# AliBahri94/GM3D

Measured on AMD Instinct MI355X. Metric: point-clouds/sec pretrain step (N=1024,G=64), higher is better.
Workload: dtype bf16

## Files before the change

### gm3d_amd/csrc/gemm_ws.hip

```cpp
#include "mfma.hpp"

namespace gm3d {

__device__ __forceinline__ void ws_wait_vm(int n) {
#define GM3D_WS_CASE(N_) case N_: asm volatile("s_waitcnt vmcnt(%0)" ::"n"(N_) : "memory"); break;
    switch (n) {
        GM3D_WS_CASE(0) GM3D_WS_CASE(4) GM3D_WS_CASE(8) GM3D_WS_CASE(12) GM3D_WS_CASE(16) GM3D_WS_CASE(24) GM3D_WS_CASE(32)
        GM3D_WS_CASE(36) GM3D_WS_CASE(48)
        default: asm volatile("s_waitcnt vmcnt(0)" ::: "memory"); break;
    }
#undef GM3D_WS_CASE
}

struct WsBn {
    const bf16_t* T;
    const float* scale;
    const float* shift;
    float* partial;
    int ldt;
    float slope;
};

constexpr int ws_depth(int ppl, int tile, int stage) {
    int d = 48 / ppl < 4 ? 48 / ppl : 4;
    while (d > 1 && (d + 1) * tile + stage > 152 * 1024) --d;
    return d;
}

template <int KT, int NW, int NL, int EPI, int TM>
__global__ __launch_bounds__(64 * (NW + NL)) void gemm_tn_ws_kernel(const bf16_t* __restrict__ A, const bf16_t* __restrict__ W,
                                                                     const float* __restrict__ bias, bf16_t* __restrict__ C, int M, int N,
                                                                     int lda, int ldw, int ldc, int tiles_n, bf16_t* __restrict__ P,
                                                                     uint8_t* __restrict__ ARG, int ldp, int bias_after_pool, WsBn bn,
                                                                     int Kreal, int pool16) {
    extern __shared__ __attribute__((aligned(16))) unsigned char wsm[];
    constexpr int BN = 32 * NW, NIMG = BN / 64 > 0 ? (BN + 63) / 64 : 1;
    constexpr int HALF = KT * 4096;
    constexpr int TILE = TM * HALF;
    constexpr int NP = TM * 4 * KT;
    constexpr int PPL = NP / NL;
    constexpr int STAGE = TM * NIMG * 4096;
    constexpr int DEPTH = ws_depth(PPL, TILE, STAGE);
    constexpr int NT = DEPTH + 1;
    static_assert(NP % NL == 0 && PPL <= 48, "loader split");
    unsigned char* stage = wsm + NT * TILE;
    const int tid = threadIdx.x, lane = tid & 63, w = __builtin_amdgcn_readfirstlane(tid >> 6);
    const int r = lane & 31, hh = lane >> 5;
    const int logical = xcd_tile(blockIdx.x, gridDim.x);
    const int tile_n = logical % tiles_n, first = logical / tiles_n, stride = gridDim.x / tiles_n;
    const int tiles_m = (M + 32 * TM - 1) / (32 * TM);
    const int nmine = first < tiles_m ? (tiles_m - first + stride - 1) / stride : 0;
    const int n0 = tile_n * BN;
    const unsigned lds0 = lds_addr(wsm);

    if (w >= NW) {
        const int lw = w - NW, prow = lane >> 3, pslot = lane & 7;
        auto issue = [&](int i) {
            const int m0 = (first + i * stride) * (32 * TM);
            const unsigned base = lds0 + (i % NT) * TILE;
#pragma unroll
            for (int q = 0; q < PPL; ++q) {
                const int p = lw * PPL + q, t = p / (4 * KT), pp = p - t * (4 * KT), kt = pp >> 2, row = 8 * (pp & 3) + prow;
                const int gr = m0 + 32 * t + row;
                const int am = gr < M ? gr : M - 1;
                int col = 64 * kt + ((pslot ^ swz(row)) << 3);
                col = col < Kreal ? col : 0;
                glds16(A + (size_t)am * lda + col, base + 1024 * p);
            }
        };
        for (int d = 0; d < DEPTH && d < nmine; ++d) issue(d);
        for (int i = 0; i < nmine; ++i) {
            if (i + DEPTH < nmine) issue(i + DEPTH);
            const int ahead = nmine - 1 - i < DEPTH ? nmine - 1 - i : DEPTH;
            ws_wait_vm(ahead * PPL);
            __builtin_amdgcn_s_barrier();
            __builtin_amdgcn_s_barrier();
        }
        return;
    }

    bf16x8 wreg[KT][4];
    {
        const bf16_t* wp = W + (size_t)(n0 + 32 * w + r) * ldw + 8 * hh;
#pragma unroll
        for (int kt = 0; kt < KT; ++kt)
#pragma unroll
            for (int s = 0; s < 4; ++s) {
                if (64 * kt + 16 * s + 8 * hh < Kreal) wreg[kt][s] = *reinterpret_cast<const bf16x8*>(wp + 64 * kt + 16 * s);
                else
#pragma unroll
                    for (int e = 0; e < 8; ++e) wreg[kt][s][e] = (bf16_t)0.0f;
            }
    }
    float bq[4][4];
#pragma unroll
    for (int q = 0; q < 4; ++q)
#pragma unroll
        for (int e = 0; e < 4; ++e) bq[q][e] = (EPI != 3 && bias) ? bias[n0 + 32 * w + 8 * q + 4 * hh + e] : 0.f;
    const float bcol = (EPI == 3 && bias) ? bias[n0 + 32 * w + r] : 0.f;
    const bool bias_in_tile = EPI != 3 || !bias_after_pool;
    float bn_a[4][4], bn_b[4][4];
    if (EPI == 4 || EPI == 5) {
#pragma unroll
        for (int q = 0; q < 4; ++q)
#pragma unroll
            for (int e = 0; e < 4; ++e) {
                const int col = n0 + 32 * w + 8 * q + 4 * hh + e;
                bn_a[q][e] = EPI == 4 ? bn.scale[col] : 0.f;
                bn_b[q][e] = EPI == 4 ? bn.shift[col] : 0.f;
            }
    }
    constexpr int CTHREADS = 64 * NW;

    for (int i = 0; i < nmine; ++i) {
        const int m0 = (first + i * stride) * (32 * TM);
        float tq[TM][4][4];
        if (EPI == 4 || EPI == 5) {
            typedef const __attribute__((address_space(4))) unsigned int* sptr_t;
#pragma unroll
            for (int t = 0; t < TM; ++t) {
                const size_t trow = pool16 ? (size_t)2 * ((m0 >> 5) + t) : (size_t)((m0 >> 5) + t);
                sptr_t tp = (sptr_t)(const void*)(bn.T + trow * bn.ldt + n0 + 32 * w);
                unsigned tw[16];
#pragma unroll
                for (int j = 0; j < 16; ++j) tw[j] = tp[j];
                if (pool16) {
                    sptr_t tp2 = (sptr_t)(const void*)(bn.T + (trow + 1) * bn.ldt + n0 + 32 * w);
                    unsigned tw2[16];
#pragma unroll
                    for (int j = 0; j < 16; ++j) tw2[j] = tp2[j];
                    if (r & 16) {
#pragma unroll
                        for (int j = 0; j < 16; ++j) tw[j] = tw2[j];
                    }
                }
#pragma unroll
                for (int q = 0; q < 4; ++q)
#pragma unroll
                    for (int e2 = 0; e2 < 2; ++e2) {
                        const unsigned u = hh ? tw[4 * q + 2 + e2] : tw[4 * q + e2];
                        tq[t][q][2 * e2] = __builtin_bit_cast(float, u << 16);
                        tq[t][q][2 * e2 + 1] = __builtin_bit_cast(float, u & 0xffff0000u);
                    }
            }
        }
        __builtin_amdgcn_s_barrier();
        const unsigned char* as = wsm + (i % NT) * TILE;
        f32x16 acc[TM];
#pragma unroll
        for (int t = 0; t < TM; ++t)
#pragma unroll
            for (int g = 0; g < 16; ++g) acc[t][g] = 0.f;
#pragma unroll
        for (int kt = 0; kt < KT; ++kt) {
            bf16x8 fa[TM][4];
#pragma unroll
            for (int t = 0; t < TM; ++t)
#pragma unroll
                for (int s = 0; s < 4; ++s) fa[t][s] = *reinterpret_cast<const bf16x8*>(as + t * HALF + kt * 4096 + swz_off(r, 2 * s + hh));
#pragma unroll
            for (int s = 0; s < 4; ++s)
#pragma unroll
                for (int t = 0; t < TM; ++t)
                    acc[t] = EPI == 3 ? mfma_bf16(fa[t][s], wreg[kt][s], acc[t])
                                      : mfma_bf16(wreg[kt][s], fa[t][s], acc[t]);
        }
        if (EPI == 3 && !C) __builtin_amdgcn_s_barrier();
        if (EPI == 3) {
            unsigned short rowbits[TM][16];
#pragma unroll
            for (int t = 0; t < TM; ++t) {
                unsigned best = 0, best2 = 0;
#pragma unroll
                for (int g = 0; g < 16; ++g) {
                    const bf16_t o = (bf16_t)(acc[t][g] + (bias_in_tile ? bcol : 0.f));
                    rowbits[t][g] = __builtin_bit_cast(unsigned short, o);
                    unsigned u = (unsigned)rowbits[t][g] << 16;
                    u = u == 0x80000000u ? 0u : u;
                    const unsigned k = (u ^ (unsigned)(((int)u >> 31) | (int)0x80000000)) & 0xffff0000u;
                    const unsigned key = k | (unsigned)(31 - (8 * (g >> 2) + 4 * hh + (g & 3)));
                    if (pool16 && g >= 8) best2 = key > best2 ? key : best2;
                    else best = key > best ? key : best;
                }
                {
                    const unsigned other = (unsigned)__shfl_xor((int)best, 32);
                    best = other > best ? other : best;
                    const unsigned other2 = (unsigned)__shfl_xor((int)best2, 32);
                    best2 = other2 > best2 ? other2 : best2;
                }
                if (hh == 0 && m0 + 32 * t < M) {
                    const unsigned k = best & 0xffff0000u;
                    const unsigned u = (k & 0x80000000u) ? (k & 0x7fff0000u) : (~k & 0xffff0000u);
                    float v = __builtin_bit_cast(float, u);
                    if (bias_after_pool) v += bcol;
                    if (!pool16) {
                        const size_t o = (size_t)((m0 >> 5) + t) * ldp + n0 + 32 * w + r;
                        P[o] = (bf16_t)v;
                        ARG[o] = (uint8_t)(31u - (best & 0xffu));
                    } else {
                        const size_t o = (size_t)((m0 >> 4) + 2 * t) * ldp + n0 + 32 * w + r;
                        P[o] = (bf16_t)v;
                        ARG[o] = (uint8_t)(31u - (best & 0xffu));
                        if (m0 + 32 * t + 16 < M) {
                            const unsigned k2 = best2 & 0xffff0000u;
                            const unsigned u2 = (k2 & 0x80000000u) ? (k2 & 0x7fff0000u) : (~k2 & 0xffff0000u);
                            float v2 = __builtin_bit_cast(float, u2);
                            if (bias_after_pool) v2 += bcol;
                            P[o + ldp] = (bf16_t)v2;
                            ARG[o + ldp] = (uint8_t)(15u - (best2 & 0xffu));
                        }
                    }
                }
            }
            if (!C) continue;
            const int ch = (((32 * w) & 63) + r) >> 3, sub = 2 * (r & 7);
#pragma unroll
            for (int t = 0; t < TM; ++t) {
                unsigned char* img = stage + (t * NIMG + ((32 * w) >> 6)) * 4096;
#pragma unroll
                for (int g = 0; g < 16; ++g) {
                    const int row = 8 * (g >> 2) + 4 * hh + (g & 3);
                    *reinterpret_cast<unsigned short*>(img + swz_off(row, ch) + sub) = rowbits[t][g];
                }
            }
        } else {
            const int cbase = ((32 * w) & 63) >> 3;
#pragma unroll
            for (int t = 0; t < TM; ++t) {
                unsigned char* img = stage + (t * NIMG + ((32 * w) >> 6)) * 4096;
#pragma unroll
                for (int q = 0; q < 4; ++q) {
                    bf16x4 pk;
#pragma unroll
                    for (int e = 0; e < 4; ++e) {
                        pk[e] = (bf16_t)(acc[t][4 * q + e] + bq[q][e]);
                        if (EPI == 4) {
                            const float h = ((float)pk[e] + tq[t][q][e]) * bn_a[q][e] + bn_b[q][e];
                            pk[e] = (bf16_t)(h > 0.f ? h : bn.slope * h);
                        }
                        if (EPI == 5) {
                            const float y = (float)pk[e] + tq[t][q][e];
                            bn_a[q][e] += y;
                            bn_b[q][e] += y * y;
                        }
                    }
                    *reinterpret_cast<bf16x4*>(img + swz_off(r, cbase + q) + 8 * hh) = pk;
                }
            }
        }
        asm volatile("s_waitcnt lgkmcnt(0)" ::: "memory");
        __builtin_amdgcn_s_barrier();
        {
            constexpr int CH = BN / 8;
#pragma unroll
            for (int c0 = 0; c0 < 32 * TM * CH; c0 += CTHREADS) {
                const int c = c0 + tid;
                if (c < 32 * TM * CH) {
                    const int row = c / CH, chunk = c - row * CH;
                    if (m0 + row < M) {
                        const uint4 raw = *reinterpret_cast<const uint4*>(stage + ((row >> 5) * NIMG + (chunk >> 3)) * 4096 + swz_off(row & 31, chunk & 7));
                        *reinterpret_cast<uint4*>(C + (size_t)(m0 + row) * ldc + n0 + 8 * chunk) = raw;
                    }
                }
            }
        }
    }
    if (EPI == 5) {
#pragma unroll
        for (int q = 0; q < 4; ++q)
#pragma unroll
            for (int e = 0; e < 4; ++e) {
#pragma unroll
                for (int m = 1; m < 32; m <<= 1) {
                    bn_a[q][e] += __shfl_xor(bn_a[q][e], m);
                    bn_b[q][e] += __shfl_xor(bn_b[q][e], m);
                }
                if (r == 0) {
                    const int col = n0 + 32 * w + 8 * q + 4 * hh + e;
                    bn.partial[(size_t)first * 2 * N + col] = bn_a[q][e];
                    bn.partial[(size_t)first * 2 * N + N + col] = bn_b[q][e];
                }
            }
    }
}

}

using gm3d::ws_depth;

static int ws_grid(int tiles_m, int tiles_n, size_t lds) {
    long long want = (long long)tiles_m * tiles_n;
    const int cap = 2 * lds <= 160 * 1024 ? 512 : 256;
    int g = want < cap ? (int)want : cap;
    g = (g + 7) / 8 * 8;
    while (g % tiles_n) g += 8;
    return g;
}

static int ws_launch(const void* A, const void* W, const float* bias, void* C, void* P, uint8_t* ARG, int M, int N, int K, int lda,
                     int ldw, int ldc, int ldp, int bias_after_pool, gm3d_stream_t stream, int bn_mode = 0, gm3d::WsBn bn = gm3d::WsBn(),
                     int pool16 = 0) {
    using namespace gm3d;
    if (!A || !W || (!C && !P) || M < 0 || N < 1 || K < 1) return GM3D_EINVAL;
    if (P && (!ARG || M % (pool16 ? 16 : 32) || ldp % 8 || ldp < N || ((size_t)ARG & 7) || ((size_t)P & 15))) return GM3D_EINVAL;
    if (K % 8 || K > 512 || lda % 8 || ldw % 8 || lda < K || ldw < K || (C && (ldc % 8 || ldc < N))) return GM3D_EUNSUPPORTED;
    if (((size_t)A | (size_t)W | (size_t)C) & 15) return GM3D_EUNSUPPORTED;
    if (M == 0) return GM3D_OK;
#define GM3D_WS_LAUNCH(KT, NW, NL, EPI, TM)                                                                               \
    {                                                                                                                    \
        constexpr int TILE_ = TM * KT * 4096, STAGE_ = TM * ((32 * NW + 63) / 64) * 4096;                                \
        constexpr int DEPTH_ = ws_depth(TM * 4 * KT / NL, TILE_, STAGE_);                                                \
        const size_t lds = (size_t)(DEPTH_ + 1) * TILE_ + STAGE_;                                                        \
        const int tiles_m = (M + 32 * TM - 1) / (32 * TM);                                                               \
        const int tiles_n = N / (32 * NW), grid = ws_grid(tiles_m, tiles_n, lds);                                        \
        return launch_lds<gemm_tn_ws_kernel<KT, NW, NL, EPI, TM>>(dim3(grid), dim3(64 * (NW + NL)), lds, stream, (const bf16_t*)A, \
                                                                  (const bf16_t*)W, bias, (bf16_t*)C, M, N, lda, ldw, ldc, tiles_n, \
                                                                  (bf16_t*)P, ARG, ldp, bias_after_pool, bn, K, pool16);        \
    }
    if (P) {
        if (K == 128 && N == 256) GM3D_WS_LAUNCH(2, 8, 1, 3, 1)
        if (K == 512 && N == 384) GM3D_WS_LAUNCH(8, 6, 2, 3, 1)
        if (K == 512 && N == 96) GM3D_WS_LAUNCH(8, 3, 2, 3, 1)
        return GM3D_EUNSUPPORTED;
    }
    if (bn_mode) {
        if (M % 32 || !bn.T || bn.ldt % 4 || bn.ldt < N || ((size_t)bn.T & 7)) return GM3D_EINVAL;
        if (K == 256 && N == 512 && bn_mode == 4) GM3D_WS_LAUNCH(4, 8, 1, 4, 1)
        if (K == 256 && N == 512 && bn_mode == 5) GM3D_WS_LAUNCH(4, 8, 1, 5, 1)
        return GM3D_EUNSUPPORTED;
    }
    if (K == 256 && N == 512) GM3D_WS_LAUNCH(4, 8, 1, 0, 1)
    if (K == 512 && N == 256) GM3D_WS_LAUNCH(8, 4, 2, 0, 1)
    if (K == 384 && N == 512) GM3D_WS_LAUNCH(6, 8, 2, 0, 1)
    if (K == 256 && N == 128) GM3D_WS_LAUNCH(4, 4, 1, 0, 1)
    if (K == 128 && N == 256) GM3D_WS_LAUNCH(2, 8, 1, 0, 1)
    if (K == 512 && N == 384) GM3D_WS_LAUNCH(8, 6, 2, 0, 1)
    if (K == 96 && N == 288) GM3D_WS_LAUNCH(2, 9, 1, 0, 1)
    if (K == 96 && N == 96) GM3D_WS_LAUNCH(2, 3, 1, 0, 1)
    if (K == 96 && N == 512) GM3D_WS_LAUNCH(2, 8, 1, 0, 1)
    if (K == 96 && N == 192) GM3D_WS_LAUNCH(2, 6, 1, 0, 1)
    if (K == 192 && N == 96) GM3D_WS_LAUNCH(3, 3, 1, 0, 1)
    if (K == 96 && N == 384) GM3D_WS_LAUNCH(2, 6, 1, 0, 1)
    if (K == 384 && N == 96) GM3D_WS_LAUNCH(6, 3, 1, 0, 1)
    if (K == 288 && N == 96) GM3D_WS_LAUNCH(5, 3, 1, 0, 1)
#undef GM3D_WS_LAUNCH
    return GM3D_EUNSUPPORTED;
}

extern "C" int gm3d_gemm_tn_bf16_ws(const void* A, const void* W, const float* bias, void* C, int M, int N, int K, int lda, int ldw,
                                    int ldc, gm3d_stream_t stream) {
    if (!C) return GM3D_EINVAL;
    return ws_launch(A, W, bias, C, nullptr, nullptr, M, N, K, lda, ldw, ldc, 0, 0, stream);
}

extern "C" int gm3d_gemm_tn_bf16_ws_pool(const void* A, const void* W, const float* bias, void* C, void* P, uint8_t* arg, int M, int N,
                                         int K, int lda, int ldw, int ldc, int ldp, int bias_after_pool, gm3d_stream_t stream) {
    if (!P || !arg) return GM3D_EINVAL;
    return ws_launch(A, W, bias, C, P, arg, M, N, K, lda, ldw, ldc, ldp, bias_after_pool, stream);
}

extern "C" int gm3d_gemm_tn_bf16_ws_poolg(const void* A, const void* W, const float* bias, void* C, void* P, uint8_t* arg, int M, int N,
                                          int K, int lda, int ldw, int ldc, int ldp, int bias_after_pool, int group_rows,
                                          gm3d_stream_t stream) {
    if (!P || !arg || (group_rows != 16 && group_rows != 32)) return GM3D_EINVAL;
    return ws_launch(A, W, bias, C, P, arg, M, N, K, lda, ldw, ldc, ldp, bias_after_pool, stream, 0, gm3d::WsBn(), group_rows == 16);
}

extern "C" int gm3d_gemm_tn_bf16_ws_bn_apply(const void* A, const void* W, const void* T, const float* scale, const float* shift, float slope,
                                             void* C, int M, int N, int K, int lda, int ldw, int ldt, int ldc, gm3d_stream_t stream) {
    if (!C || !T || !scale || !shift) return GM3D_EINVAL;
    gm3d::WsBn bn;
    bn.T = (const gm3d::bf16_t*)T; bn.scale = scale; bn.shift = shift; bn.partial = nullptr; bn.ldt = ldt; bn.slope = slope;
    return ws_launch(A, W, nullptr, C, nullptr, nullptr, M, N, K, lda, ldw, ldc, 0, 0, stream, 4, bn);
}

extern "C" int gm3d_gemm_tn_bf16_ws_bn_stats(const void* A, const void* W, const void* T, void* C, float* partial, int M, int N, int K,
                                             int lda, int ldw, int ldt, int ldc, gm3d_stream_t stream) {
    if (!C || !T || !partial) return GM3D_EINVAL;
    gm3d::WsBn bn;
    bn.T = (const gm3d::bf16_t*)T; bn.scale = nullptr; bn.shift = nullptr; bn.partial = partial; bn.ldt = ldt; bn.slope = 0.f;
    return ws_launch(A, W, nullptr, C, nullptr, nullptr, M, N, K, lda, ldw, ldc, 0, 0, stream, 5, bn);
}

extern "C" int gm3d_gemm_tn_bf16_ws_bn_apply_g(const void* A, const void* W, const void* T, const float* scale, const float* shift, float slope,
                                               void* C, int M, int N, int K, int lda, int ldw, int ldt, int ldc, int group_rows,
                                               gm3d_stream_t stream) {
    if (!C || !T || !scale || !shift || (group_rows != 16 && group_rows != 32)) return GM3D_EINVAL;
    gm3d::WsBn bn;
    bn.T = (const gm3d::bf16_t*)T; bn.scale = scale; bn.shift = shift; bn.partial = nullptr; bn.ldt = ldt; bn.slope = slope;
    return ws_launch(A, W, nullptr, C, nullptr, nullptr, M, N, K, lda, ldw, ldc, 0, 0, stream, 4, bn, group_rows == 16);
}

extern "C" int gm3d_gemm_tn_bf16_ws_bn_stats_g(const void* A, const void* W, const void* T, void* C, float* partial, int M, int N, int K,
                                               int lda, int ldw, int ldt, int ldc, int group_rows, gm3d_stream_t stream) {
    if (!C || !T || !partial || (group_rows != 16 && group_rows != 32)) return GM3D_EINVAL;
    gm3d::WsBn bn;
    bn.T = (const gm3d::bf16_t*)T; bn.scale = nullptr; bn.shift = nullptr; bn.partial = partial; bn.ldt = ldt; bn.slope = 0.f;
    return ws_launch(A, W, nullptr, C, nullptr, nullptr, M, N, K, lda, ldw, ldc, 0, 0, stream, 5, bn, group_rows == 16);
}

extern "C" int gm3d_gemm_ws_stats_rows(int M, int N, int K) {
    if (!(K == 256 && N == 512) || M % 32 || M < 32) return 0;
    constexpr int KT = 4, NW = 8, NL = 1;
    constexpr int TILE_ = KT * 4096, STAGE_ = ((32 * NW + 63) / 64) * 4096;
    const size_t lds = (size_t)(ws_depth(4 * KT / NL, TILE_, STAGE_) + 1) * TILE_ + STAGE_;
    const int tiles_n = N / (32 * NW);
    return ws_grid(M / 32, tiles_n, lds) / tiles_n;
}

extern "C" int gm3d_gemm_ws_supported(int N, int K, int pool) {
    if (pool) return (K == 128 && N == 256) || (K == 512 && N == 384) || (K == 512 && N == 96);
    return (K == 256 && N == 512) || (K == 512 && N == 256) || (K == 384 && N == 512) || (K == 256 && N == 128) ||
           (K == 128 && N == 256) || (K == 512 && N == 384) || (K == 96 && (N == 288 || N == 96 || N == 384 || N == 192 || N == 512)) || (K == 384 && N == 96) ||
           (K == 288 && N == 96) || (K == 192 && N == 96);
}
```

### gm3d_amd/csrc/mfma.hpp

```cpp
#pragma once
#include "common.hpp"

namespace gm3d {

typedef __bf16 bf16x8 __attribute__((ext_vector_type(8)));
typedef __bf16 bf16x4 __attribute__((ext_vector_type(4)));
typedef float f32x16 __attribute__((ext_vector_type(16)));
typedef __attribute__((address_space(3))) bf16x4 lds_bf16x4;

__device__ __forceinline__ f32x16 mfma_bf16(bf16x8 a, bf16x8 b, f32x16 c) {
    return __builtin_amdgcn_mfma_f32_32x32x16_bf16(a, b, c, 0, 0, 0);
}

__device__ __forceinline__ f32x16 mfma_f32(float a, float b, f32x16 c) { return __builtin_amdgcn_mfma_f32_32x32x2f32(a, b, c, 0, 0, 0); }

__device__ __forceinline__ int crow(int g, int hh) { return (g & 3) + 8 * (g >> 2) + 4 * hh; }

__device__ __forceinline__ bf16x8 zero8() {
    bf16x8 z;
#pragma unroll
    for (int j = 0; j < 8; ++j) z[j] = (bf16_t)0.0f;
    return z;
}
__device__ __forceinline__ f32x16 zero16() {
    f32x16 z;
#pragma unroll
    for (int g = 0; g < 16; ++g) z[g] = 0.f;
    return z;
}
__device__ __forceinline__ bf16x8 cvt8(const f32x16& x, int s, float mul) {
    bf16x8 v;
#pragma unroll
    for (int j = 0; j < 8; ++j) v[j] = (bf16_t)(x[8 * s + j] * mul);
    return v;
}

__device__ __forceinline__ int swz(int row) { return (((row >> 1) & 1) << 2) | (((row >> 2) & 1) << 1) | ((row >> 3) & 1); }
__device__ __forceinline__ int swz_off(int row, int ch) { return row * 128 + ((ch ^ swz(row)) << 4); }

__device__ __forceinline__ unsigned lds_addr(const unsigned char* p) {
    return (unsigned)(size_t)(__attribute__((address_space(3))) const unsigned char*)p;
}

__device__ __forceinline__ void glds16(const void* gsrc, unsigned dst) {
    unsigned keep;
    asm volatile("s_mov_b32 %0, m0\n\ts_mov_b32 m0, %2\n\ts_nop 0\n\tglobal_load_lds_dwordx4 %1, off\n\ts_mov_b32 m0, %0"
                 : "=&s"(keep)
                 : "v"(gsrc), "s"(dst)
                 : "memory");
}

template <class I> __device__ __forceinline__ int xcd_tile(I block, I grid) {
    const int per_xcd = grid >> 3;
    return (block & 7) * per_xcd + (block >> 3);
}

}
```

Measured before the change: 16940.

## Add store warps, ring-loaded BN T rows, and software-pipelined LDS fragment loads

Adds dedicated store wavefronts (for KT=4, NW=8 shapes) that drain a double-buffered output stage to global memory while compute warps move on to the next tile. BN-mode T rows now arrive through the loader ring via global_load_lds_dword instead of scalar loads in the compute warps. The MFMA inner loop prefetches LDS fragments WS_PF steps ahead with sched_barriers. These changes aim to hide store latency and T-row load latency behind MFMA work, at the cost of more LDS, more threads per block, and a more complex barrier protocol.

New measurement: 17020 (median of 6 runs). Within noise of the previous version (+0.4%).

```diff
diff --git a/gm3d_amd/csrc/gemm_ws.hip b/gm3d_amd/csrc/gemm_ws.hip
--- a/gm3d_amd/csrc/gemm_ws.hip
+++ b/gm3d_amd/csrc/gemm_ws.hip
@@ -5,8 +5,8 @@
 __device__ __forceinline__ void ws_wait_vm(int n) {
 #define GM3D_WS_CASE(N_) case N_: asm volatile("s_waitcnt vmcnt(%0)" ::"n"(N_) : "memory"); break;
     switch (n) {
-        GM3D_WS_CASE(0) GM3D_WS_CASE(4) GM3D_WS_CASE(8) GM3D_WS_CASE(12) GM3D_WS_CASE(16) GM3D_WS_CASE(24) GM3D_WS_CASE(32)
-        GM3D_WS_CASE(36) GM3D_WS_CASE(48)
+        GM3D_WS_CASE(0) GM3D_WS_CASE(4) GM3D_WS_CASE(8) GM3D_WS_CASE(12) GM3D_WS_CASE(16) GM3D_WS_CASE(20) GM3D_WS_CASE(24)
+        GM3D_WS_CASE(32) GM3D_WS_CASE(36) GM3D_WS_CASE(40) GM3D_WS_CASE(48) GM3D_WS_CASE(60)
         default: asm volatile("s_waitcnt vmcnt(0)" ::: "memory"); break;
     }
 #undef GM3D_WS_CASE
@@ -21,18 +21,20 @@
     float slope;
 };
 
+constexpr int WS_PF = 4;
+
 constexpr int ws_depth(int ppl, int tile, int stage) {
     int d = 48 / ppl < 4 ? 48 / ppl : 4;
     while (d > 1 && (d + 1) * tile + stage > 152 * 1024) --d;
     return d;
 }
 
-template <int KT, int NW, int NL, int EPI, int TM>
-__global__ __launch_bounds__(64 * (NW + NL)) void gemm_tn_ws_kernel(const bf16_t* __restrict__ A, const bf16_t* __restrict__ W,
-                                                                     const float* __restrict__ bias, bf16_t* __restrict__ C, int M, int N,
-                                                                     int lda, int ldw, int ldc, int tiles_n, bf16_t* __restrict__ P,
-                                                                     uint8_t* __restrict__ ARG, int ldp, int bias_after_pool, WsBn bn,
-                                                                     int Kreal, int pool16) {
+template <int KT, int NW, int NL, int EPI, int TM, int NS>
+__global__ __launch_bounds__(64 * (NW + NL + NS)) void gemm_tn_ws_kernel(const bf16_t* __restrict__ A, const bf16_t* __restrict__ W,
+                                                                          const float* __restrict__ bias, bf16_t* __restrict__ C, int M,
+                                                                          int N, int lda, int ldw, int ldc, int tiles_n,
+                                                                          bf16_t* __restrict__ P, uint8_t* __restrict__ ARG, int ldp,
+                                                                          int bias_after_pool, WsBn bn, int Kreal, int pool16) {
     extern __shared__ __attribute__((aligned(16))) unsigned char wsm[];
     constexpr int BN = 32 * NW, NIMG = BN / 64 > 0 ? (BN + 63) / 64 : 1;
     constexpr int HALF = KT * 4096;
@@ -42,8 +44,15 @@
     constexpr int STAGE = TM * NIMG * 4096;
     constexpr int DEPTH = ws_depth(PPL, TILE, STAGE);
     constexpr int NT = DEPTH + 1;
-    static_assert(NP % NL == 0 && PPL <= 48, "loader split");
+    constexpr bool BNT = EPI == 4 || EPI == 5;
+    constexpr int NSTG = NS ? 2 : 1;
+    constexpr int TP = BNT ? 4 : 0;
+    constexpr int TAREA = 256 * TP;
+    static_assert(NP % NL == 0 && PPL <= 48 && DEPTH * (PPL + TP) <= 63, "loader split");
+    static_assert(!BNT || (BN == 256 && TM == 1), "T rows ride the ring as four 256-byte pieces");
+    static_assert(NT * TILE + NSTG * STAGE + NT * TAREA <= 160 * 1024, "LDS");
     unsigned char* stage = wsm + NT * TILE;
+    unsigned char* tarea = stage + NSTG * STAGE;
     const int tid = threadIdx.x, lane = tid & 63, w = __builtin_amdgcn_readfirstlane(tid >> 6);
     const int r = lane & 31, hh = lane >> 5;
     const int logical = xcd_tile(blockIdx.x, gridDim.x);
@@ -53,7 +62,7 @@
     const int n0 = tile_n * BN;
     const unsigned lds0 = lds_addr(wsm);
 
-    if (w >= NW) {
+    if (w >= NW && w < NW + NL) {
         const int lw = w - NW, prow = lane >> 3, pslot = lane & 7;
         auto issue = [&](int i) {
             const int m0 = (first + i * stride) * (32 * TM);
@@ -67,14 +76,62 @@
                 col = col < Kreal ? col : 0;
                 glds16(A + (size_t)am * lda + col, base + 1024 * p);
             }
+            if (BNT && lw == 0) {
+                const int g = m0 >> 5, nrows = pool16 ? M >> 4 : M >> 5;
+#pragma unroll
+                for (int j = 0; j < TP; ++j) {
+                    int trow = pool16 ? 2 * g + (j >> 1) : g;
+                    trow = trow < nrows ? trow : nrows - 1;
+                    glds4(bn.T + (size_t)trow * bn.ldt + n0 + 128 * (j & 1) + 2 * lane, lds_addr(tarea) + (i % NT) * TAREA + 256 * j);
+                }
+            }
         };
+        const int ppl = PPL + (lw == 0 ? TP : 0);
         for (int d = 0; d < DEPTH && d < nmine; ++d) issue(d);
         for (int i = 0; i < nmine; ++i) {
             if (i + DEPTH < nmine) issue(i + DEPTH);
             const int ahead = nmine - 1 - i < DEPTH ? nmine - 1 - i : DEPTH;
-            ws_wait_vm(ahead * PPL);
+            ws_wait_vm(ahead * ppl);
             __builtin_amdgcn_s_barrier();
             __builtin_amdgcn_s_barrier();
+        }
+        return;
+    }
+    constexpr int CH = BN / 8;
+    if (NS && w >= NW + NL) {
+        constexpr int STHREADS = 64 * (NS ? NS : 1), PER = 32 * TM * CH / STHREADS;
+        static_assert(32 * TM * CH % STHREADS == 0, "store split");
+        if (!C) {
+            for (int i = 0; i < 2 * nmine; ++i) __builtin_amdgcn_s_barrier();
+            return;
+        }
+        const int st = tid - 64 * (NW + NL);
+        int soff[PER], srow[PER];
+        size_t coff[PER];
+#pragma unroll
+        for (int k = 0; k < PER; ++k) {
+            const int c = k * STHREADS + st, row = c / CH, chunk = c - row * CH;
+            soff[k] = ((row >> 5) * NIMG + (chunk >> 3)) * 4096 + swz_off(row & 31, chunk & 7);
+            srow[k] = row;
+            coff[k] = (size_t)row * ldc + n0 + 8 * chunk;
+        }
+        uint4 held[PER];
+#pragma unroll
+        for (int k = 0; k < PER; ++k) held[k] = make_uint4(0, 0, 0, 0);
+        for (int i = 0; i <= nmine; ++i) {
+            if (i < nmine) __builtin_amdgcn_s_barrier();
+            if (i > 0) {
+                const int m0 = (first + (i - 1) * stride) * (32 * TM);
+#pragma unroll
+                for (int k = 0; k < PER; ++k)
+                    if (m0 + srow[k] < M) *reinterpret_cast<uint4*>(C + (size_t)m0 * ldc + coff[k]) = held[k];
+            }
+            if (i == nmine) break;
+            asm volatile("s_waitcnt lgkmcnt(0)" ::: "memory");
+            __builtin_amdgcn_s_barrier();
+            const unsigned char* sg = stage + (i & 1) * STAGE;
+#pragma unroll
+            for (int k = 0; k < PER; ++k) held[k] = *reinterpret_cast<const uint4*>(sg + soff[k]);
         }
         return;
     }
@@ -96,7 +153,7 @@
 #pragma unroll
     for (int q = 0; q < 4; ++q)
 #pragma unroll
-        for (int e = 0; e < 4; ++e) bq[q][e] = (EPI != 3 && bias) ? bias[n0 + 32 * w + 8 * q + 4 * hh + e] : 0.f;
+        for (int e = 0; e < 4; ++e) bq[q][e] = (EPI != 3 && !BNT && bias) ? bias[n0 + 32 * w + 8 * q + 4 * hh + e] : 0.f;
     const float bcol = (EPI == 3 && bias) ? bias[n0 + 32 * w + r] : 0.f;
     const bool bias_in_tile = EPI != 3 || !bias_after_pool;
     float bn_a[4][4], bn_b[4][4];
@@ -114,56 +171,42 @@
 
     for (int i = 0; i < nmine; ++i) {
         const int m0 = (first + i * stride) * (32 * TM);
+        __builtin_amdgcn_s_barrier();
         float tq[TM][4][4];
-        if (EPI == 4 || EPI == 5) {
-            typedef const __attribute__((address_space(4))) unsigned int* sptr_t;
-#pragma unroll
-            for (int t = 0; t < TM; ++t) {
-                const size_t trow = pool16 ? (size_t)2 * ((m0 >> 5) + t) : (size_t)((m0 >> 5) + t);
-                sptr_t tp = (sptr_t)(const void*)(bn.T + trow * bn.ldt + n0 + 32 * w);
-                unsigned tw[16];
-#pragma unroll
-                for (int j = 0; j < 16; ++j) tw[j] = tp[j];
-                if (pool16) {
-                    sptr_t tp2 = (sptr_t)(const void*)(bn.T + (trow + 1) * bn.ldt + n0 + 32 * w);
-                    unsigned tw2[16];
-#pragma unroll
-                    for (int j = 0; j < 16; ++j) tw2[j] = tp2[j];
-                    if (r & 16) {
-#pragma unroll
-                        for (int j = 0; j < 16; ++j) tw[j] = tw2[j];
-                    }
-                }
-#pragma unroll
-                for (int q = 0; q < 4; ++q)
-#pragma unroll
-                    for (int e2 = 0; e2 < 2; ++e2) {
-                        const unsigned u = hh ? tw[4 * q + 2 + e2] : tw[4 * q + e2];
-                        tq[t][q][2 * e2] = __builtin_bit_cast(float, u << 16);
-                        tq[t][q][2 * e2 + 1] = __builtin_bit_cast(float, u & 0xffff0000u);
-                    }
-            }
-        }
-        __builtin_amdgcn_s_barrier();
+        if (BNT) {
+            const unsigned char* ts = tarea + (i % NT) * TAREA + (pool16 ? (r >> 4) * (2 * BN) : 0) + 2 * (32 * w + 4 * hh);
+#pragma unroll
+            for (int q = 0; q < 4; ++q) {
+                const bf16x4 tv = *reinterpret_cast<const bf16x4*>(ts + 16 * q);
+#pragma unroll
+                for (int e = 0; e < 4; ++e) tq[0][q][e] = (float)tv[e];
+            }
+        }
         const unsigned char* as = wsm + (i % NT) * TILE;
         f32x16 acc[TM];
 #pragma unroll
         for (int t = 0; t < TM; ++t)
 #pragma unroll
             for (int g = 0; g < 16; ++g) acc[t][g] = 0.f;
-#pragma unroll
-        for (int kt = 0; kt < KT; ++kt) {
-            bf16x8 fa[TM][4];
-#pragma unroll
-            for (int t = 0; t < TM; ++t)
-#pragma unroll
-                for (int s = 0; s < 4; ++s) fa[t][s] = *reinterpret_cast<const bf16x8*>(as + t * HALF + kt * 4096 + swz_off(r, 2 * s + hh));
-#pragma unroll
-            for (int s = 0; s < 4; ++s)
-#pragma unroll
-                for (int t = 0; t < TM; ++t)
-                    acc[t] = EPI == 3 ? mfma_bf16(fa[t][s], wreg[kt][s], acc[t])
-                                      : mfma_bf16(wreg[kt][s], fa[t][s], acc[t]);
+        constexpr int NSTEP = 4 * KT;
+        auto frag = [&](int t, int j) {
+            return *reinterpret_cast<const bf16x8*>(as + t * HALF + (j >> 2) * 4096 + swz_off(r, 2 * (j & 3) + hh));
+        };
+        bf16x8 fa[TM][WS_PF];
+#pragma unroll
+        for (int j = 0; j < WS_PF; ++j)
+#pragma unroll
+            for (int t = 0; t < TM; ++t) fa[t][j] = frag(t, j);
+        __builtin_amdgcn_sched_barrier(0);
+#pragma unroll
+        for (int j = 0; j < NSTEP; ++j) {
+#pragma unroll
+            for (int t = 0; t < TM; ++t) {
+                acc[t] = EPI == 3 ? mfma_bf16(fa[t][j % WS_PF], wreg[j >> 2][j & 3], acc[t])
+                                  : mfma_bf16(wreg[j >> 2][j & 3], fa[t][j % WS_PF], acc[t]);
+                if (j + WS_PF < NSTEP) fa[t][j % WS_PF] = frag(t, j + WS_PF);
+            }
+            __builtin_amdgcn_sched_barrier(0);
         }
         if (EPI == 3 && !C) __builtin_amdgcn_s_barrier();
         if (EPI == 3) {
@@ -216,7 +259,7 @@
             const int ch = (((32 * w) & 63) + r) >> 3, sub = 2 * (r & 7);
 #pragma unroll
             for (int t = 0; t < TM; ++t) {
-                unsigned char* img = stage + (t * NIMG + ((32 * w) >> 6)) * 4096;
+                unsigned char* img = stage + (NS ? (i & 1) * STAGE : 0) + (t * NIMG + ((32 * w) >> 6)) * 4096;
 #pragma unroll
                 for (int g = 0; g < 16; ++g) {
                     const int row = 8 * (g >> 2) + 4 * hh + (g & 3);
@@ -227,7 +270,7 @@
             const int cbase = ((32 * w) & 63) >> 3;
 #pragma unroll
             for (int t = 0; t < TM; ++t) {
-                unsigned char* img = stage + (t * NIMG + ((32 * w) >> 6)) * 4096;
+                unsigned char* img = stage + (NS ? (i & 1) * STAGE : 0) + (t * NIMG + ((32 * w) >> 6)) * 4096;
 #pragma unroll
                 for (int q = 0; q < 4; ++q) {
                     bf16x4 pk;
@@ -250,8 +293,7 @@
         }
         asm volatile("s_waitcnt lgkmcnt(0)" ::: "memory");
         __builtin_amdgcn_s_barrier();
-        {
-            constexpr int CH = BN / 8;
+        if (!NS) {
 #pragma unroll
             for (int c0 = 0; c0 < 32 * TM * CH; c0 += CTHREADS) {
                 const int c = c0 + tid;
@@ -287,6 +329,10 @@
 }
 
 using gm3d::ws_depth;
+
+constexpr int ws_ns(int kt, int nw, int epi) {
+    return kt == 4 && nw == 8 ? 2 : 0;
+}
 
 static int ws_grid(int tiles_m, int tiles_n, size_t lds) {
     long long want = (long long)tiles_m * tiles_n;
@@ -309,13 +355,15 @@
 #define GM3D_WS_LAUNCH(KT, NW, NL, EPI, TM)                                                                               \
     {                                                                                                                    \
         constexpr int TILE_ = TM * KT * 4096, STAGE_ = TM * ((32 * NW + 63) / 64) * 4096;                                \
-        constexpr int DEPTH_ = ws_depth(TM * 4 * KT / NL, TILE_, STAGE_);                                                \
-        const size_t lds = (size_t)(DEPTH_ + 1) * TILE_ + STAGE_;                                                        \
+        constexpr int DEPTH_ = ws_depth(TM * 4 * KT / NL, TILE_, STAGE_), NS_ = ws_ns(KT, NW, EPI);                      \
+        const size_t ring = (size_t)(DEPTH_ + 1) * TILE_ + STAGE_;                                                       \
+        const size_t lds = ring + (NS_ ? STAGE_ : 0) + ((EPI == 4 || EPI == 5) ? (DEPTH_ + 1) * 1024 : 0);               \
         const int tiles_m = (M + 32 * TM - 1) / (32 * TM);                                                               \
-        const int tiles_n = N / (32 * NW), grid = ws_grid(tiles_m, tiles_n, lds);                                        \
-        return launch_lds<gemm_tn_ws_kernel<KT, NW, NL, EPI, TM>>(dim3(grid), dim3(64 * (NW + NL)), lds, stream, (const bf16_t*)A, \
-                                                                  (const bf16_t*)W, bias, (bf16_t*)C, M, N, lda, ldw, ldc, tiles_n, \
-                                                                  (bf16_t*)P, ARG, ldp, bias_after_pool, bn, K, pool16);        \
+        const int tiles_n = N / (32 * NW), grid = ws_grid(tiles_m, tiles_n, ring);                                       \
+        return launch_lds<gemm_tn_ws_kernel<KT, NW, NL, EPI, TM, NS_>>(dim3(grid), dim3(64 * (NW + NL + NS_)), lds, stream,         \
+                                                                       (const bf16_t*)A, (const bf16_t*)W, bias, (bf16_t*)C, M, N, lda, \
+                                                                       ldw, ldc, tiles_n, (bf16_t*)P, ARG, ldp, bias_after_pool, bn, K, \
+                                                                       pool16);                                                      \
     }
     if (P) {
         if (K == 128 && N == 256) GM3D_WS_LAUNCH(2, 8, 1, 3, 1)
diff --git a/gm3d_amd/csrc/mfma.hpp b/gm3d_amd/csrc/mfma.hpp
--- a/gm3d_amd/csrc/mfma.hpp
+++ b/gm3d_amd/csrc/mfma.hpp
@@ -50,6 +50,14 @@
                  : "memory");
 }
 
+__device__ __forceinline__ void glds4(const void* gsrc, unsigned dst) {
+    unsigned keep;
+    asm volatile("s_mov_b32 %0, m0\n\ts_mov_b32 m0, %2\n\ts_nop 0\n\tglobal_load_lds_dword %1, off\n\ts_mov_b32 m0, %0"
+                 : "=&s"(keep)
+                 : "v"(gsrc), "s"(dst)
+                 : "memory");
+}
+
 template <class I> __device__ __forceinline__ int xcd_tile(I block, I grid) {
     const int per_xcd = grid >> 3;
     return (block & 7) * per_xcd + (block >> 3);
```
